# navi0105/LyricAlignment

Hardware: AMD Instinct MI355X
Metric: aligned audio-sec/sec (RTF^-1), Whisper-medium 30 s clips (higher is better)
Workload: dtype bf16; 1 GPU; whisper-medium encoder + BiGRU/FC head + CTC forced alignment, batch 32 x 30 s mel per GPU (BASELINE.json configs[1]); clips_per_gpu=32, frames=1500, vocab=21129, labels_per_clip=5..26 (one per sung note), pipeline=2 encoder stream(s) + 1 head stream, head over 4 batches

## Files before the change

### lyricalignment_amd/csrc/la_attention.hip

```cpp
#include <type_traits>

#include "la_common.h"

using la::bf16_t;

namespace {

typedef __attribute__((ext_vector_type(16))) float f32x16;
typedef __attribute__((ext_vector_type(8))) __bf16 bf16x8;
typedef __attribute__((ext_vector_type(8))) _Float16 f16x8;

template <typename T16> struct Half16;
template <> struct Half16<bf16_t> {
    typedef bf16x8 vec8;
    typedef __bf16 elem;
    static constexpr unsigned kOnes = 0x3F803F80u;
    static constexpr float kPLimit = 0x1p30f;
    __device__ static __forceinline__ f32x16 mfma32(vec8 a, vec8 b, f32x16 c) { return __builtin_amdgcn_mfma_f32_32x32x16_bf16(a, b, c, 0, 0, 0); }
};
template <> struct Half16<la::f16_t> {
    typedef f16x8 vec8;
    typedef _Float16 elem;
    static constexpr unsigned kOnes = 0x3C003C00u;
    static constexpr float kPLimit = 0x1p13f;
    __device__ static __forceinline__ f32x16 mfma32(vec8 a, vec8 b, f32x16 c) { return __builtin_amdgcn_mfma_f32_32x32x16_f16(a, b, c, 0, 0, 0); }
};
typedef __attribute__((ext_vector_type(4))) short s16x4;

constexpr int QT = 128;
constexpr int KT = 64;
constexpr float kLog2e = 1.4426950408889634f;

struct AttnParams {
    const void *q, *k, *v;
    int64_t ld_q, ld_kv;
    void *out;
    int64_t ld_out;
    int q_len, kv_len, n_head, causal;
    int64_t q_bs, kv_bs, out_bs;
    int batch;
    float defer_thr;
    float *lse = nullptr;
    float score_scale = 1.4426950408889634f;
};

struct BlockCoord { int qt, head, clip; };
__device__ __forceinline__ BlockCoord block_coord(int nq, int n_head, int batch) {
    const int L = blockIdx.x, pairs = n_head * batch;
    int pair, qt;
    if ((pairs & 7) == 0) {
        const int x = L & 7, idx = L >> 3;
        pair = x + 8 * (idx / nq);
        qt = idx % nq;
    } else {
        pair = L / nq;
        qt = L % nq;
    }
    return BlockCoord{qt, pair % n_head, pair / n_head};
}

__device__ __forceinline__ int acc_row(int reg, int h) { return (reg & 3) + 8 * (reg >> 2) + 4 * h; }

__device__ __forceinline__ void glds16(const void *g, void *l) {
    la::glds16(g, l);
}

__device__ __forceinline__ int kswz(int r) { return (r >> 1) & 7; }
__device__ __forceinline__ int vswz(int r) { return ((r >> 1) & 1) << 2; }

struct KvOff { unsigned k[2], v[2]; };
template <int PER>
__device__ __forceinline__ KvOff kv_offsets_bf16(int64_t ld, int key0, int T, int wave, int lane) {
    KvOff o;
    const int r8 = lane >> 3, ps = lane & 7;
#pragma unroll
    for (int i = 0; i < PER; ++i) {
        const int r = (wave * PER + i) * 8 + r8;
        int rr = key0 + r < T ? r : T - 1 - key0;
        o.k[i] = (unsigned)(rr * ld * 2) + ((ps ^ kswz(r)) << 4);
        o.v[i] = (unsigned)(rr * ld * 2) + ((ps ^ vswz(r)) << 4);
    }
    return o;
}
template <int PER>
__device__ __forceinline__ void stage_kv_bf16(const bf16_t *kbase, const bf16_t *vbase, int64_t ld, int key0, const KvOff &o,
                                              unsigned kl, unsigned vl, int wave) {
    const bf16_t *ks = kbase + (int64_t)key0 * ld, *vs = vbase + (int64_t)key0 * ld;
#pragma unroll
    for (int i = 0; i < PER; ++i) {
        la::glds16_so(o.k[i], ks, kl + (wave * PER + i) * 1024);
        la::glds16_so(o.v[i], vs, vl + (wave * PER + i) * 1024);
    }
}

template <typename T16, int NW = 4, bool MSUM = false, int KO = 0, bool OPT = false, int PRIO = 0, bool FOLD = false>
__global__ __launch_bounds__(64 * NW, FOLD ? 4 : 2) void attention_bf16_kernel(AttnParams p) {
    static_assert(!(OPT && MSUM), "the optimistic form tests the vector-pipe row sums");
    static_assert(!FOLD || OPT, "the log2-domain form is a variant of the optimistic one");
    constexpr int QT = 32 * NW, PER = 8 / NW;
    typedef Half16<T16> HT;
    typedef typename HT::vec8 vec8;
    __shared__ __attribute__((aligned(16))) unsigned char lds[2 * 2 * KT * 128];
    const int T = p.kv_len;
    const BlockCoord bc = block_coord((p.q_len + QT - 1) / QT, p.n_head, p.batch);
    const int qt = bc.qt, head = bc.head, clip = bc.clip;
    const int tid = threadIdx.x, lane = tid & 63;
    const int wave = __builtin_amdgcn_readfirstlane(tid >> 6);
    const int i32 = lane & 31, h = lane >> 5;
    const bf16_t *base = reinterpret_cast<const bf16_t *>(p.q) + (int64_t)clip * p.q_bs * p.ld_q + head * 64;
    const bf16_t *kbase = reinterpret_cast<const bf16_t *>(p.k) + (int64_t)clip * p.kv_bs * p.ld_kv + head * 64;
    const bf16_t *vbase = reinterpret_cast<const bf16_t *>(p.v) + (int64_t)clip * p.kv_bs * p.ld_kv + head * 64;

    int qrow = qt * QT + wave * 32 + i32;
    const bool q_valid = qrow < p.q_len;
    qrow = q_valid ? qrow : p.q_len - 1;
    uint4 qf[4];
#pragma unroll
    for (int c = 0; c < 4; ++c) qf[c] = *reinterpret_cast<const uint4 *>(base + (int64_t)qrow * p.ld_q + 16 * c + 8 * h);

    f32x16 o[2];
#pragma unroll
    for (int b = 0; b < 2; ++b)
#pragma unroll
        for (int r = 0; r < 16; ++r) o[b][r] = 0.f;
    float m_run = FOLD ? 0.f : -INFINITY, l_part = 0.f;
    int plain = FOLD ? 1 : 0;
    const float kScale = FOLD ? 1.0f : p.score_scale;
    f32x16 osum;
#pragma unroll
    for (int r = 0; r < 16; ++r) osum[r] = 0.f;
    const uint4 ones4 = uint4{HT::kOnes, HT::kOnes, HT::kOnes, HT::kOnes};

    int nkv = (T + KT - 1) / KT;
    const int nkv_all = nkv;
    if (p.causal) nkv = min(nkv, (min(p.q_len, (qt + 1) * QT) - 1) / KT + 1);
    const unsigned lds0 = __builtin_amdgcn_readfirstlane(la::lds_addr_u32(lds));
    const KvOff off_full = kv_offsets_bf16<PER>(p.ld_kv, 0, KT, wave, lane);
    const KvOff off_last = kv_offsets_bf16<PER>(p.ld_kv, (nkv_all - 1) * KT, T, wave, lane);
    stage_kv_bf16<PER>(kbase, vbase, p.ld_kv, 0, nkv_all == 1 ? off_last : off_full, lds0, lds0 + KT * 128, wave);
    asm volatile("s_waitcnt vmcnt(0)" ::: "memory");
#pragma unroll
    for (int c = 0; c < 4; ++c) {
        typedef unsigned u32x4 __attribute__((ext_vector_type(4)));
        u32x4 t = __builtin_bit_cast(u32x4, qf[c]);
        asm volatile("" : "+v"(t));
        qf[c] = __builtin_bit_cast(uint4, t);
    }
    __syncthreads();

    const int g = lane >> 4, q4 = (lane & 15) >> 2, pp = lane & 3;

    auto tile = [&](int t, auto curc) __attribute__((always_inline)) {
        constexpr int cur = decltype(curc)::value;
        const unsigned char *kl = lds + cur * (2 * KT * 128);
        const unsigned char *vl = kl + KT * 128;
        if (t + 1 < nkv && !(KO & 8)) {
            const unsigned nk = lds0 + (cur ^ 1) * (2 * KT * 128);
            stage_kv_bf16<PER>(kbase, vbase, p.ld_kv, (t + 1) * KT, t + 2 == nkv_all ? off_last : off_full, nk, nk + KT * 128, wave);
        }
        f32x16 s[2];
        typedef std::integral_constant<int, 0> Sub0;
        typedef std::integral_constant<int, 1> Sub1;
        typedef std::integral_constant<int, 2> SubBoth;
        auto scores = [&](auto serialc, auto whichc) {
            constexpr bool serial = decltype(serialc)::value;
            constexpr int lo = decltype(whichc)::value == 2 ? 0 : decltype(whichc)::value;
            constexpr int hi = decltype(whichc)::value == 2 ? 2 : lo + 1;
            uint4 kf[2][4];
#pragma unroll
            for (int sub = lo; sub < hi; ++sub)
#pragma unroll
                for (int r = 0; r < 16; ++r) s[sub][r] = 0.f;
            if constexpr (!serial) {
#pragma unroll
                for (int c = 0; c < 4; ++c)
#pragma unroll
                    for (int sub = lo; sub < hi; ++sub) {
                        const int row = sub * 32 + i32;
                        if constexpr (KO & 4) kf[sub][c] = qf[(c + sub) & 3];
                        else kf[sub][c] = *reinterpret_cast<const uint4 *>(kl + row * 128 + (((2 * c + h) ^ kswz(row)) << 4));
                    }
            }
#pragma unroll
            for (int c = 0; c < 4; ++c) {
                if constexpr (serial) {
#pragma unroll
                    for (int sub = lo; sub < hi; ++sub) {
                        const int row = sub * 32 + i32;
                        kf[sub][c] = *reinterpret_cast<const uint4 *>(kl + row * 128 + (((2 * c + h) ^ kswz(row)) << 4));
                    }
                }
// ... 65 lines not shown
#pragma unroll
                for (int j = 0; j < 8; ++j) pf[j] = (typename HT::elem)s[sub][8 * ks + j];
                if constexpr (MSUM) osum = HT::mfma32(__builtin_bit_cast(vec8, ones4), pf, osum);
#pragma unroll
                for (int b = 0; b < 2; ++b) {
                    const int key0 = sub * 32 + 16 * ks + 4 * (g >> 1);
                    const int slot = b * 4 + 2 * (g & 1) + (pp >> 1);
                    const int r0 = key0 + q4, r1 = key0 + 8 + q4;
                    typedef __attribute__((ext_vector_type(8))) short s16x8;
                    s16x8 vf;
                    if constexpr (KO & 2) vf = __builtin_bit_cast(s16x8, qf[(2 * sub + ks + b) & 3]);
                    else {
                        const s16x4 v0 = __builtin_amdgcn_ds_read_tr16_b64_v4i16(
                            (__attribute__((address_space(3))) s16x4 *)(vl + r0 * 128 + ((slot ^ vswz(r0)) << 4) + (pp & 1) * 8));
                        const s16x4 v1 = __builtin_amdgcn_ds_read_tr16_b64_v4i16(
                            (__attribute__((address_space(3))) s16x4 *)(vl + r1 * 128 + ((slot ^ vswz(r1)) << 4) + (pp & 1) * 8));
                        vf = __builtin_shufflevector(v0, v1, 0, 1, 2, 3, 4, 5, 6, 7);
                    }
                    if constexpr (KO & 16) o[b][2 * sub + ks] += (float)vf[0] + (float)vf[7] + (float)pf[0] + (float)pf[7];
                    else o[b] = HT::mfma32(__builtin_bit_cast(vec8, vf), pf, o[b]);
                }
            }
        };
        auto redo = [&](auto whichc) -> float {
            scores(std::true_type{}, whichc);
            const float m_new = fmaxf(m_run, tile_max(whichc));
            const float alpha = __builtin_amdgcn_exp2f(m_run - m_new);
            m_run = m_new;
            plain = 0;
            rescale(alpha);
            l_part *= alpha;
            return exponentials(m_new, whichc);
        };
        if constexpr (PRIO == 1 || PRIO == 2) __builtin_amdgcn_s_setprio(3);
        scores(std::false_type{}, SubBoth{});
        if constexpr (PRIO == 1 || PRIO == 2) __builtin_amdgcn_s_setprio(0);
        if constexpr (PRIO == 3) __builtin_amdgcn_s_setprio(3);
        if constexpr (OPT) {
            float ps0 = exponentials(m_run, Sub0{});
            if (__builtin_expect(__builtin_amdgcn_ballot_w64(!(ps0 <= HT::kPLimit)) != 0, 0)) ps0 = redo(Sub0{});
            l_part += ps0;
            float ps1 = exponentials(m_run, Sub1{});
            pv_sub(Sub0{});
            if (__builtin_expect(__builtin_amdgcn_ballot_w64(!(ps1 <= HT::kPLimit)) != 0, 0)) ps1 = redo(Sub1{});
            l_part += ps1;
            if constexpr (PRIO == 3) __builtin_amdgcn_s_setprio(0);
            if constexpr (PRIO == 2) __builtin_amdgcn_s_setprio(3);
            pv_sub(Sub1{});
            if constexpr (PRIO == 2) __builtin_amdgcn_s_setprio(0);
        } else {
            const float mx2 = tile_max(SubBoth{});
            float m_new = m_run, alpha = 1.0f;
            if (__builtin_amdgcn_ballot_w64(mx2 > m_run + p.defer_thr) != 0) {
                m_new = fmaxf(m_run, mx2);
                alpha = __builtin_amdgcn_exp2f(m_run - m_new);
            }
            m_run = m_new;
            const float ps = exponentials(m_new, SubBoth{});
            if constexpr (!MSUM) l_part = l_part * alpha + ps;
            if (__builtin_amdgcn_ballot_w64(alpha != 1.0f) != 0) rescale(alpha);
            pv_sub(Sub0{});
            pv_sub(Sub1{});
        }
        asm volatile("s_waitcnt vmcnt(0)" ::: "memory");
        if constexpr (!(KO & 32)) __syncthreads();
    };
    auto sweep = [&]() __attribute__((always_inline)) {
        for (int t = 0; t < nkv; t += 2) {
            tile(t, std::integral_constant<int, 0>{});
            if (t + 1 < nkv) tile(t + 1, std::integral_constant<int, 1>{});
        }
    };
    sweep();
    if constexpr (FOLD) {
        const float l0 = l_part + __shfl_xor(l_part, 32);
        if (__builtin_amdgcn_readfirstlane(__syncthreads_or(q_valid && !(l0 >= 0x1p-100f && l0 <= 0x1p100f)))) {
#pragma unroll
            for (int b = 0; b < 2; ++b)
#pragma unroll
                for (int r = 0; r < 16; ++r) o[b][r] = 0.f;
            m_run = -INFINITY; l_part = 0.f; plain = 0;
            stage_kv_bf16<PER>(kbase, vbase, p.ld_kv, 0, nkv_all == 1 ? off_last : off_full, lds0, lds0 + KT * 128, wave);
            asm volatile("s_waitcnt vmcnt(0)" ::: "memory");
            __syncthreads();
            sweep();
        }
    }

    const float l = MSUM ? osum[0] : l_part + __shfl_xor(l_part, 32);
    const float inv = 1.0f / l;
    if (q_valid) {
        bf16_t *orow = reinterpret_cast<bf16_t *>(p.out) + ((int64_t)clip * p.out_bs + qrow) * p.ld_out + head * 64;
#pragma unroll
        for (int b = 0; b < 2; ++b)
#pragma unroll
            for (int r4 = 0; r4 < 4; ++r4) {
                *reinterpret_cast<ushort4 *>(orow + 32 * b + 8 * r4 + 4 * h) =
                    la::Pack4<T16>::run(o[b][4 * r4 + 0] * inv, o[b][4 * r4 + 1] * inv, o[b][4 * r4 + 2] * inv, o[b][4 * r4 + 3] * inv);
            }
    }
}

__device__ __forceinline__ void stage_kv_f32(const float *kbase, const float *vbase, int64_t ld, int key0, int T,
                                             unsigned char *kl, unsigned char *vl, int wave, int lane) {
    const int r4 = lane >> 4, ps = lane & 15;
#pragma unroll
    for (int i = 0; i < 4; ++i) {
        const int piece = wave * 4 + i;
        const int r = piece * 4 + r4;
        int key = key0 + r;
        key = key < T ? key : T - 1;
        const int ls = ps ^ (r & 15);
        glds16(kbase + (int64_t)key * ld + (ls << 2), kl + piece * 1024);
        glds16(vbase + (int64_t)key * ld + (ls << 2), vl + piece * 1024);
    }
}
// ... 97 lines not shown
                }
            }
        asm volatile("s_waitcnt vmcnt(0)" ::: "memory");
        __syncthreads();
        cur ^= 1;
    }

    const float l = l_part + __shfl_xor(l_part, 32);
    const float inv = 1.0f / l;
    if (p.lse && q_valid && h == 0)
        p.lse[((int64_t)clip * p.n_head + head) * p.q_len + qrow] = fmaf(m_run, 0.6931471805599453f, __logf(l));
    if (q_valid) {
        float *orow = reinterpret_cast<float *>(p.out) + ((int64_t)clip * p.out_bs + qrow) * p.ld_out + head * 64;
#pragma unroll
        for (int b = 0; b < 2; ++b)
#pragma unroll
            for (int r4 = 0; r4 < 4; ++r4)
                *reinterpret_cast<float4 *>(orow + 32 * b + 8 * r4 + 4 * h) =
                    make_float4(o[b][4 * r4 + 0] * inv, o[b][4 * r4 + 1] * inv, o[b][4 * r4 + 2] * inv, o[b][4 * r4 + 3] * inv);
    }
}

}

static int attention_launch(int dtype_arg, AttnParams p, int batch, hipStream_t stream) {
    const int dtype = dtype_arg & 0xff;
    const bool qlog2 = dtype_arg & LA_Q_LOG2;
    if (qlog2 && dtype != LA_BF16 && dtype != LA_F16) {
        la::set_error("attention: LA_Q_LOG2 goes with the 16-bit kernels");
        return LA_EINVAL;
    }
    p.score_scale = qlog2 ? 1.0f : kLog2e;
    p.batch = batch;
    const char *thr_env = la::dev_env("LA_ATTN_THR");
    p.defer_thr = thr_env ? (float)atof(thr_env) : 8.0f;
    const dim3 grid(la::cdiv(p.q_len, QT) * p.n_head * batch), block(256);
    if (dtype == LA_BF16 || dtype == LA_F16) {
        la::TimerScope ts("attention_bf16", stream);
        const int nw_opt = la::opts().attn_nw;
        const int nw = nw_opt ? nw_opt : (p.q_len >= 1024 ? 8 : 4);
        const dim3 grid8(la::cdiv(p.q_len, 256) * p.n_head * batch), block8(512);
        const bool wide = nw == 8 && p.q_len >= 256;
#ifdef LA_EXPERIMENTS
        const char *opt_env = getenv("LA_ATTN_OPT"), *fold_env = getenv("LA_ATTN_FOLD");
        const bool no_opt = opt_env && atoi(opt_env) == 0, no_fold = fold_env && atoi(fold_env) == 0;
        if (wide && no_opt) {
            if (dtype == LA_F16) hipLaunchKernelGGL((attention_bf16_kernel<la::f16_t, 8>), grid8, block8, 0, stream, p);
            else hipLaunchKernelGGL((attention_bf16_kernel<bf16_t, 8>), grid8, block8, 0, stream, p);
        } else if (wide && dtype == LA_BF16 && qlog2 && no_fold) {
            hipLaunchKernelGGL((attention_bf16_kernel<bf16_t, 8, false, 0, true>), grid8, block8, 0, stream, p);
        } else if (!wide && getenv("LA_ATTN_MSUM")) {
            if (dtype == LA_F16) hipLaunchKernelGGL((attention_bf16_kernel<la::f16_t, 4, true>), grid, block, 0, stream, p);
            else hipLaunchKernelGGL((attention_bf16_kernel<bf16_t, 4, true>), grid, block, 0, stream, p);
        } else if (!wide && no_opt) {
            if (dtype == LA_F16) hipLaunchKernelGGL((attention_bf16_kernel<la::f16_t, 4>), grid, block, 0, stream, p);
            else hipLaunchKernelGGL((attention_bf16_kernel<bf16_t, 4>), grid, block, 0, stream, p);
        } else if (!wide && dtype == LA_BF16 && qlog2 && no_fold) {
            hipLaunchKernelGGL((attention_bf16_kernel<bf16_t, 4, false, 0, true>), grid, block, 0, stream, p);
        } else
#endif
#ifdef LA_ATTN_KNOCKOUT
        if (const char *ko = getenv("LA_ATTN_KO"); ko && !wide) {
            switch (atoi(ko)) {
#define LA_KO_CASE(n) case n: hipLaunchKernelGGL((attention_bf16_kernel<bf16_t, 4, false, n>), grid, block, 0, stream, p); break;
                LA_KO_CASE(1) LA_KO_CASE(2) LA_KO_CASE(4) LA_KO_CASE(6) LA_KO_CASE(8) LA_KO_CASE(14) LA_KO_CASE(16) LA_KO_CASE(17)
                LA_KO_CASE(7) LA_KO_CASE(15) LA_KO_CASE(30)
#undef LA_KO_CASE
#define LA_KO_OPT(n, ko) case n: { const char *pad = getenv("LA_ATTN_LDSPAD"); \
        hipLaunchKernelGGL((attention_bf16_kernel<bf16_t, 4, false, ko, true>), grid, block, pad ? atoi(pad) : 0, stream, p); } break;
                LA_KO_OPT(132, 32) LA_KO_OPT(140, 40) LA_KO_OPT(100, 0) LA_KO_OPT(101, 1) LA_KO_OPT(106, 6) LA_KO_OPT(108, 8) LA_KO_OPT(114, 14) LA_KO_OPT(116, 16) LA_KO_OPT(130, 30)
#undef LA_KO_OPT
#define LA_KO_PRIO(n, pr) case n: hipLaunchKernelGGL((attention_bf16_kernel<bf16_t, 4, false, 0, true, pr>), grid, block, 0, stream, p); break;
                LA_KO_PRIO(201, 1) LA_KO_PRIO(202, 2) LA_KO_PRIO(203, 3)
#undef LA_KO_PRIO
                default: hipLaunchKernelGGL((attention_bf16_kernel<bf16_t, 4>), grid, block, 0, stream, p);
            }
        } else
#endif
        if (wide) {
            if (dtype == LA_F16) hipLaunchKernelGGL((attention_bf16_kernel<la::f16_t, 8, false, 0, true>), grid8, block8, 0, stream, p);
            else if (qlog2) hipLaunchKernelGGL((attention_bf16_kernel<bf16_t, 8, false, 0, true, 0, true>), grid8, block8, 0, stream, p);
            else hipLaunchKernelGGL((attention_bf16_kernel<bf16_t, 8, false, 0, true>), grid8, block8, 0, stream, p);
        } else if (dtype == LA_F16) hipLaunchKernelGGL((attention_bf16_kernel<la::f16_t, 4, false, 0, true>), grid, block, 0, stream, p);
        else if (qlog2) hipLaunchKernelGGL((attention_bf16_kernel<bf16_t, 4, false, 0, true, 0, true>), grid, block, 0, stream, p);
        else hipLaunchKernelGGL((attention_bf16_kernel<bf16_t, 4, false, 0, true>), grid, block, 0, stream, p);
    } else {
        static la::DeviceOnce attr_once;
        if (attr_once.pending()) {
            LA_HIP(hipFuncSetAttribute(reinterpret_cast<const void *>(attention_f32_kernel),
                                       hipFuncAttributeMaxDynamicSharedMemorySize, 4 * KT * 256));
            attr_once.mark();
        }
        la::TimerScope ts("attention_f32", stream);
        hipLaunchKernelGGL(attention_f32_kernel, grid, block, 4 * KT * 256, stream, p);
    }
    LA_LAUNCH_CHECK();
    return LA_OK;
}

extern "C" int la_attention(int32_t dtype_arg, const void *qkv, int64_t ld_qkv, void *out, int64_t ld_out, int32_t batch,
                            int32_t frames, int32_t n_head, void *stream_) {
    hipStream_t stream = (hipStream_t)stream_;
    if (batch == 0 || frames == 0) return LA_OK;
    LA_CHECK_ARG(qkv && out && batch > 0 && frames > 0 && n_head > 0, "attention: bad arguments");
    const int dtype = dtype_arg & 0xff;
    LA_CHECK_ARG((dtype_arg & ~(0xff | LA_Q_LOG2)) == 0 && (dtype == LA_F32 || dtype == LA_BF16 || dtype == LA_F16), "attention: bad dtype");
    const int es = dtype == LA_F32 ? 4 : 2;
    LA_CHECK_ARG(ld_qkv >= 3 * n_head * 64 && ld_out >= n_head * 64, "attention: leading dimensions too small");
    LA_CHECK_ARG((ld_qkv * es) % 16 == 0 && (ld_out * es) % 16 == 0 && (uintptr_t)qkv % 16 == 0 && (uintptr_t)out % 16 == 0,
                 "attention: rows must be 16-byte aligned");
    const char *b = reinterpret_cast<const char *>(qkv);
    const int d = n_head * 64;
    AttnParams p{b, b + (int64_t)d * es, b + (int64_t)2 * d * es, ld_qkv, ld_qkv, out, ld_out, frames, frames, n_head, 0, frames, frames, frames, 0};
    return attention_launch(dtype_arg, p, batch, stream);
}

extern "C" int la_attention_ex(int32_t dtype_arg, const void *q, int64_t ld_q, const void *k, const void *v, int64_t ld_kv,
                               void *out, int64_t ld_out, int32_t batch, int32_t q_len, int32_t kv_len, int32_t n_head,
// ... 49 lines not shown
```

### lyricalignment_amd/csrc/la_common.h

```cpp
#pragma once
#include <hip/hip_runtime.h>
#include <stdint.h>
#include <stdio.h>
#include <stdlib.h>
#include <string.h>

#include "../../include/lyricalign.h"

namespace la {

char *err_buf();
void set_error(const char *fmt, ...);

enum { SCRATCH_SPLITK = 0, SCRATCH_COLSUM = 1, SCRATCH_X2 = 2 };
void *stream_scratch(hipStream_t stream, int purpose, size_t bytes);

#define LA_CHECK_ARG(cond, ...)                \
    do {                                       \
        if (!(cond)) {                         \
            la::set_error(__VA_ARGS__);        \
            return LA_EINVAL;                  \
        }                                      \
    } while (0)

#define LA_HIP(expr)                                                                     \
    do {                                                                                 \
        hipError_t _e = (expr);                                                          \
        if (_e != hipSuccess) {                                                          \
            la::set_error("%s:%d %s -> %s", __FILE__, __LINE__, #expr, hipGetErrorString(_e)); \
            return LA_EHIP;                                                              \
        }                                                                                \
    } while (0)

#define LA_LAUNCH_CHECK()                                                               \
    do {                                                                                \
        hipError_t _e = hipGetLastError();                                              \
        if (_e != hipSuccess) {                                                         \
            la::set_error("%s:%d launch -> %s", __FILE__, __LINE__, hipGetErrorString(_e)); \
            return LA_EHIP;                                                             \
        }                                                                               \
    } while (0)

struct Options {
    int gemm_tile = 0, gemm_loop = 0, gemm_splitk = 1, attn_nw = 0, gru_nw = 0, gru_fence = 0, gru_handoff = 0, gru_poll_delay = 0, viterbi_dpp = 1,
        head_clip_cap = 0, ln_fusion = 1, resid_split = 1, x2_inference = 1, gru_timeout_us = 0, gru_fault_step = 0, x2_small = 0;
};
Options &opts();
#ifdef LA_EXPERIMENTS
inline const char *dev_env(const char *name) { return getenv(name); }
#define LA_DEV_BIT(word, bits) ((word) & (bits))
#else
inline const char *dev_env(const char *) { return nullptr; }
#define LA_DEV_BIT(word, bits) false
#endif

struct DeviceOnce {
    unsigned long long done[4] = {0, 0, 0, 0};
    static int current() {
        int d = 0;
        if (hipGetDevice(&d) != hipSuccess) d = 0;
        return d & 255;
    }
    bool pending() const {
        const int d = current();
        return !((__atomic_load_n(&done[d >> 6], __ATOMIC_ACQUIRE) >> (d & 63)) & 1ull);
    }
    void mark() {
        const int d = current();
        __atomic_fetch_or(&done[d >> 6], 1ull << (d & 63), __ATOMIC_RELEASE);
    }
};

struct TimerScope {
    bool active;
    hipStream_t stream;
    TimerScope(const char *family, hipStream_t s, double work = 0.0);
    ~TimerScope();
};
// ... 178 lines not shown
```

### lyricalignment_amd/csrc/la_elementwise.hip

```cpp
#include "la_common.h"

using la::bf16_t;

namespace {

__device__ __forceinline__ float wave_max(float v) {
#pragma unroll
    for (int o = 32; o > 0; o >>= 1) v = fmaxf(v, __shfl_xor(v, o));
    return v;
}
__device__ __forceinline__ float wave_sum(float v) {
#pragma unroll
    for (int o = 32; o > 0; o >>= 1) v += __shfl_xor(v, o);
    return v;
}

__global__ __launch_bounds__(256) void emissions_from_logits_kernel(
    const float *logits, int64_t bs, int64_t rs, int frames, int vocab, int variant, const int32_t *labels,
    int labels_stride, const int32_t *n_labels, int max_labels, float *em, int64_t em_bs, int64_t em_rs) {
    __shared__ float red[8];
    const int row = blockIdx.x;
    const int b = row / frames, t = row % frames;
    const float *x = logits + (int64_t)b * bs + (int64_t)t * rs;
    const int c0 = variant == LA_VARIANT_CTC ? 1 : 0;
// ... 149 lines not shown
template <typename T16, int MAXV>
__global__ __launch_bounds__(256) void row_stats16_kernel(const T16 *x, int64_t ldx, int M, int d, float eps, float2 *stats) {
    const int row = blockIdx.x * 4 + (threadIdx.x >> 6);
    const int lane = threadIdx.x & 63;
    if (row >= M) return;
    const T16 *xr = x + (int64_t)row * ldx;
    float v[MAXV][8];
    float sum = 0.f;
#pragma unroll
    for (int i = 0; i < MAXV; ++i) {
        const int c = (lane + 64 * i) * 8;
        if (c < d) {
            const uint4 raw = *reinterpret_cast<const uint4 *>(xr + c);
            const T16 *e = reinterpret_cast<const T16 *>(&raw);
#pragma unroll
            for (int j = 0; j < 8; ++j) { v[i][j] = la::Elem<T16>::load(e + j); sum += v[i][j]; }
        } else {
#pragma unroll
            for (int j = 0; j < 8; ++j) v[i][j] = 0.f;
        }
    }
    const float mean = wave_sum(sum) / (float)d;
    float sq = 0.f;
#pragma unroll
    for (int i = 0; i < MAXV; ++i) {
        const int c = (lane + 64 * i) * 8;
        if (c < d) {
#pragma unroll
            for (int j = 0; j < 8; ++j) { const float a = v[i][j] - mean; sq = fmaf(a, a, sq); }
        }
    }
    const float var = wave_sum(sq) / (float)d;
    if (lane == 0) stats[row] = make_float2(mean, 1.0f / sqrtf(var + eps));
}

__global__ void cast_f32_bf16_kernel(const float *x, bf16_t *y, int64_t n) {
    int64_t i = ((int64_t)blockIdx.x * blockDim.x + threadIdx.x) * 4;
    const int64_t stride = (int64_t)gridDim.x * blockDim.x * 4;
    for (; i + 3 < n; i += stride) {
        const float4 v = *reinterpret_cast<const float4 *>(x + i);
        ushort4 pk;
        pk.x = la::f32_to_bf16(v.x); pk.y = la::f32_to_bf16(v.y);
        pk.z = la::f32_to_bf16(v.z); pk.w = la::f32_to_bf16(v.w);
        *reinterpret_cast<ushort4 *>(y + i) = pk;
    }
    if (blockIdx.x == 0 && threadIdx.x == 0)
        for (int64_t j = n & ~(int64_t)3; j < n; ++j) y[j] = la::f32_to_bf16(x[j]);
}

__global__ void cast_bf16_f32_kernel(const bf16_t *x, float *y, int64_t n) {
    int64_t i = (int64_t)blockIdx.x * blockDim.x + threadIdx.x;
    const int64_t stride = (int64_t)gridDim.x * blockDim.x;
    for (; i < n; i += stride) y[i] = la::bf16_to_f32(x[i]);
}

template <typename TOut>
__global__ __launch_bounds__(256) void mel_to_rows_kernel(const float *mel, int64_t mbs, int64_t mrs, int n_mels,
                                                          int frames, TOut *out, int c_pad) {
    __shared__ float tile[32][33];
    const int b = blockIdx.z;
    const int t0 = blockIdx.x * 32;
    const int c0 = blockIdx.y * 32;
    const int tx = threadIdx.x & 31, ty = threadIdx.x >> 5;
    for (int i = ty; i < 32; i += 8) {
        const int c = c0 + i, r = t0 + tx;
        const int t = r - 1;
// ... 84 lines not shown
    const unsigned char *l = reinterpret_cast<const unsigned char *>(lo);
    if (out_dtype == LA_F32)
        hipLaunchKernelGGL((layernorm_split_kernel<T16, float, 8>), grid, block, 0, stream, h, l, ldx, M, d, gamma, beta, (float *)y, ldy);
    else if (out_dtype == LA_F16)
        hipLaunchKernelGGL((layernorm_split_kernel<T16, la::f16_t, 8>), grid, block, 0, stream, h, l, ldx, M, d, gamma, beta, (la::f16_t *)y, ldy);
    else
        hipLaunchKernelGGL((layernorm_split_kernel<T16, bf16_t, 8>), grid, block, 0, stream, h, l, ldx, M, d, gamma, beta, (bf16_t *)y, ldy);
    LA_LAUNCH_CHECK();
    return LA_OK;
}

extern "C" int la_layernorm_split(int32_t dtype, const void *hi, const void *lo, int64_t ldx, int32_t M, int32_t d, const float *gamma,
                                  const float *beta, void *y, int64_t ldy, int32_t out_dtype, void *stream_) {
    hipStream_t stream = (hipStream_t)stream_;
    if (M == 0) return LA_OK;
    LA_CHECK_ARG(hi && lo && gamma && beta && y, "layernorm_split: null pointer");
    LA_CHECK_ARG(dtype == LA_BF16 || dtype == LA_F16, "layernorm_split: the stream's hi part is bf16 or f16");
    LA_CHECK_ARG(d > 0 && d % 4 == 0 && d <= 64 * 4 * 8 && ldx % 4 == 0 && ldy % 4 == 0 && (uintptr_t)hi % 8 == 0 && (uintptr_t)lo % 4 == 0,
                 "layernorm_split: d=%d unsupported or misaligned rows", d);
    LA_CHECK_ARG(out_dtype == LA_F32 || out_dtype == LA_BF16 || out_dtype == LA_F16, "layernorm_split: bad dtype");
    la::TimerScope ts("layernorm", stream);
    return dtype == LA_F16 ? layernorm_split_launch<la::f16_t>(hi, lo, ldx, M, d, gamma, beta, y, ldy, out_dtype, stream)
                           : layernorm_split_launch<bf16_t>(hi, lo, ldx, M, d, gamma, beta, y, ldy, out_dtype, stream);
}

extern "C" int la_row_stats16(int32_t dtype, const void *x, int64_t ldx, int32_t M, int32_t d, float eps, float *stats, void *stream_) {
    if (M == 0) return LA_OK;
    LA_CHECK_ARG(x && stats && M > 0 && d > 0, "row_stats16: bad arguments");
    LA_CHECK_ARG(dtype == LA_BF16 || dtype == LA_F16, "row_stats16: 16-bit rows only");
    LA_CHECK_ARG(d % 8 == 0 && d <= 64 * 8 * 4 && ldx % 8 == 0 && ((uintptr_t)x % 16 == 0) && ((uintptr_t)stats % 8 == 0),
                 "row_stats16: d must be a multiple of 8 and <= 2048, rows 16-byte aligned");
    hipStream_t stream = (hipStream_t)stream_;
    la::TimerScope ts("layernorm", stream);
    const dim3 grid(la::cdiv(M, 4)), block(256);
    if (dtype == LA_F16)
        hipLaunchKernelGGL((row_stats16_kernel<la::f16_t, 4>), grid, block, 0, stream, (const la::f16_t *)x, ldx, M, d, eps, (float2 *)stats);
    else
        hipLaunchKernelGGL((row_stats16_kernel<bf16_t, 4>), grid, block, 0, stream, (const bf16_t *)x, ldx, M, d, eps, (float2 *)stats);
    LA_LAUNCH_CHECK();
    return LA_OK;
}

extern "C" int la_cast_f32_to_bf16(const float *x, void *y, int64_t n, void *stream_) {
    if (n == 0) return LA_OK;
    LA_CHECK_ARG(x && y && n > 0, "cast: bad arguments");
    LA_CHECK_ARG(((uintptr_t)x % 16 == 0) && ((uintptr_t)y % 8 == 0), "cast: pointers must be 16/8-byte aligned");
    const int grid = (int)std::min<int64_t>(2048, la::cdiv(n, 1024));
    hipLaunchKernelGGL(cast_f32_bf16_kernel, dim3(grid), dim3(256), 0, (hipStream_t)stream_, x, (bf16_t *)y, n);
    LA_LAUNCH_CHECK();
    return LA_OK;
}

extern "C" int la_cast_bf16_to_f32(const void *x, float *y, int64_t n, void *stream_) {
    if (n == 0) return LA_OK;
    LA_CHECK_ARG(x && y && n > 0, "cast: bad arguments");
    const int grid = (int)std::min<int64_t>(2048, la::cdiv(n, 256));
    hipLaunchKernelGGL(cast_bf16_f32_kernel, dim3(grid), dim3(256), 0, (hipStream_t)stream_, (const bf16_t *)x, y, n);
    LA_LAUNCH_CHECK();
    return LA_OK;
}

extern "C" int la_mel_to_rows(const float *mel, int64_t mel_batch_stride, int64_t mel_row_stride, int32_t batch,
                              int32_t n_mels, int32_t frames, void *out, int32_t c_pad, int32_t dtype, void *stream_) {
    if (batch == 0) return LA_OK;
    LA_CHECK_ARG(mel && out && batch > 0 && n_mels > 0 && frames > 0 && c_pad >= n_mels, "mel_to_rows: bad arguments");
    LA_CHECK_ARG(dtype == LA_F32 || dtype == LA_BF16 || dtype == LA_F16, "mel_to_rows: bad dtype");
    const dim3 grid(la::cdiv(frames + 2, 32), la::cdiv(c_pad, 32), batch), block(256);
    hipStream_t stream = (hipStream_t)stream_;
    if (dtype == LA_F32)
        hipLaunchKernelGGL((mel_to_rows_kernel<float>), grid, block, 0, stream, mel, mel_batch_stride, mel_row_stride,
                           n_mels, frames, (float *)out, c_pad);
// ... 100 lines not shown
```

### lyricalignment_amd/csrc/la_runtime.cpp

```cpp
#include <stdarg.h>
#include <stdlib.h>

#include <mutex>
#include <string>
#include <vector>

#include "la_common.h"

namespace la {

char *err_buf() {
    static thread_local char buf[512] = {0};
    return buf;
}

void set_error(const char *fmt, ...) {
    va_list ap;
    va_start(ap, fmt);
    vsnprintf(err_buf(), 512, fmt, ap);
    va_end(ap);
}

void *stream_scratch(hipStream_t stream, int purpose, size_t bytes) {
    struct Slot { int dev; hipStream_t stream; int purpose; void *ptr; size_t bytes; };
    static std::mutex mu;
    static std::vector<Slot> slots;
    int dev = 0;
    if (hipGetDevice(&dev) != hipSuccess) return nullptr;
    std::lock_guard<std::mutex> lock(mu);
    for (Slot &sl : slots)
        if (sl.dev == dev && sl.stream == stream && sl.purpose == purpose) {
            if (sl.bytes >= bytes) return sl.ptr;
            if (hipStreamSynchronize(stream) != hipSuccess) return nullptr;
            (void)hipFree(sl.ptr);
            sl.ptr = nullptr; sl.bytes = 0;
            if (hipMalloc(&sl.ptr, bytes) != hipSuccess) return nullptr;
            sl.bytes = bytes;
            return sl.ptr;
        }
    Slot sl{dev, stream, purpose, nullptr, bytes < ((size_t)1 << 20) ? ((size_t)1 << 20) : bytes};
    if (hipMalloc(&sl.ptr, sl.bytes) != hipSuccess) return nullptr;
    slots.push_back(sl);
    return sl.ptr;
}

namespace {
struct OptionDesc { const char *name, *env; int Options::*field; bool env_inverts; };
const OptionDesc kOptions[] = {
    {"gemm_tile", "LA_GEMM_TILE", &Options::gemm_tile, false},       {"gemm_loop", "LA_PP_DBG", &Options::gemm_loop, false},
    {"gemm_splitk", "LA_GEMM_NO_SPLITK", &Options::gemm_splitk, true}, {"attn_nw", "LA_ATTN_NW", &Options::attn_nw, false},
    {"gru_nw", "LA_GRU_NW", &Options::gru_nw, false},                 {"gru_fence", "LA_GRU_FENCE", &Options::gru_fence, false},
    {"gru_handoff", "LA_GRU_HANDOFF", &Options::gru_handoff, false}, {"gru_poll_delay", "LA_GRU_POLL_DELAY", &Options::gru_poll_delay, false},
    {"viterbi_dpp", "LA_VITERBI_NO_DPP", &Options::viterbi_dpp, true}, {"head_clip_cap", "LA_HEAD_CLIP_CAP", &Options::head_clip_cap, false},
    {"ln_fusion", "LA_LN_FUSION", &Options::ln_fusion, false},       {"resid_split", "LA_RESID_SPLIT", &Options::resid_split, false},
    {"x2_inference", "LA_X2_INFERENCE", &Options::x2_inference, false}, {"x2_small", "LA_X2_SMALL", &Options::x2_small, false},
    {"gru_timeout_us", "LA_GRU_TIMEOUT_US", &Options::gru_timeout_us, false}, {"gru_fault_step", "LA_GRU_FAULT_STEP", &Options::gru_fault_step, false},
};
}

Options &opts() {
    static Options o = [] {
        Options v;
        for (const OptionDesc &d : kOptions) {
            const char *e = getenv(d.env);
            if (!e) continue;
            v.*(d.field) = d.env_inverts ? 0 : atoi(e);
        }
        return v;
    }();
    return o;
}

namespace {
struct TimerState {
    std::mutex mu;
    bool enabled = false;
    std::string family;
    std::vector<std::pair<hipEvent_t, hipEvent_t>> pairs;
    std::vector<std::pair<hipEvent_t, hipEvent_t>> pool;
    int period = 1;
    int64_t seen = 0;
    double work = 0.0;
};
TimerState &ts() {
    static TimerState s;
    return s;
}
}

// ... 135 lines not shown
```

Before: 23640 audio-sec/sec.

## Skip dead query waves and half-empty last KV tile in attention; add optional ring buffer

Attention waves whose query rows all lie past q_len now only take part in staging and barriers and skip score, softmax and PV work. When the final KV tile holds at most 32 valid keys, only its first 32-key half is computed. Both are on by default and aim to remove padded work at the sequence tails, which matters for the 1500-frame encoder. Two opt-in paths are added but stay off by default: a three-slot LDS ring for K/V prefetch with partial vmcnt waits, and a multi-row LayerNorm statistics kernel. The extra template modes increase code size and add branches.

```diff
diff --git a/lyricalignment_amd/csrc/la_attention.hip b/lyricalignment_amd/csrc/la_attention.hip
--- a/lyricalignment_amd/csrc/la_attention.hip
+++ b/lyricalignment_amd/csrc/la_attention.hip
@@ -42,6 +42,7 @@
     float defer_thr;
     float *lse = nullptr;
     float score_scale = 1.4426950408889634f;
+    int tails = 1;
 };
 
 struct BlockCoord { int qt, head, clip; };
@@ -93,14 +94,15 @@
     }
 }
 
-template <typename T16, int NW = 4, bool MSUM = false, int KO = 0, bool OPT = false, int PRIO = 0, bool FOLD = false>
+template <typename T16, int NW = 4, bool MSUM = false, int KO = 0, bool OPT = false, int PRIO = 0, bool FOLD = false, int RING = 2>
 __global__ __launch_bounds__(64 * NW, FOLD ? 4 : 2) void attention_bf16_kernel(AttnParams p) {
     static_assert(!(OPT && MSUM), "the optimistic form tests the vector-pipe row sums");
     static_assert(!FOLD || OPT, "the log2-domain form is a variant of the optimistic one");
+    static_assert(RING == 2 || RING == 3, "double buffer or ring of three");
     constexpr int QT = 32 * NW, PER = 8 / NW;
     typedef Half16<T16> HT;
     typedef typename HT::vec8 vec8;
-    __shared__ __attribute__((aligned(16))) unsigned char lds[2 * 2 * KT * 128];
+    __shared__ __attribute__((aligned(16))) unsigned char lds[RING * 2 * KT * 128];
     const int T = p.kv_len;
     const BlockCoord bc = block_coord((p.q_len + QT - 1) / QT, p.n_head, p.batch);
     const int qt = bc.qt, head = bc.head, clip = bc.clip;
@@ -114,6 +116,7 @@
     int qrow = qt * QT + wave * 32 + i32;
     const bool q_valid = qrow < p.q_len;
     qrow = q_valid ? qrow : p.q_len - 1;
+    const bool live = !p.tails || qt * QT + wave * 32 < p.q_len;
     uint4 qf[4];
 #pragma unroll
     for (int c = 0; c < 4; ++c) qf[c] = *reinterpret_cast<const uint4 *>(base + (int64_t)qrow * p.ld_q + 16 * c + 8 * h);
@@ -137,8 +140,13 @@
     const unsigned lds0 = __builtin_amdgcn_readfirstlane(la::lds_addr_u32(lds));
     const KvOff off_full = kv_offsets_bf16<PER>(p.ld_kv, 0, KT, wave, lane);
     const KvOff off_last = kv_offsets_bf16<PER>(p.ld_kv, (nkv_all - 1) * KT, T, wave, lane);
-    stage_kv_bf16<PER>(kbase, vbase, p.ld_kv, 0, nkv_all == 1 ? off_last : off_full, lds0, lds0 + KT * 128, wave);
-    asm volatile("s_waitcnt vmcnt(0)" ::: "memory");
+    auto prologue = [&]() __attribute__((always_inline)) {
+        stage_kv_bf16<PER>(kbase, vbase, p.ld_kv, 0, nkv_all == 1 ? off_last : off_full, lds0, lds0 + KT * 128, wave);
+        if (RING == 3 && nkv > 1)
+            stage_kv_bf16<PER>(kbase, vbase, p.ld_kv, KT, nkv_all == 2 ? off_last : off_full, lds0 + 2 * KT * 128, lds0 + 3 * KT * 128, wave);
+        asm volatile("s_waitcnt vmcnt(0)" ::: "memory");
+    };
+    prologue();
 #pragma unroll
     for (int c = 0; c < 4; ++c) {
         typedef unsigned u32x4 __attribute__((ext_vector_type(4)));
@@ -150,13 +158,20 @@
 
     const int g = lane >> 4, q4 = (lane & 15) >> 2, pp = lane & 3;
 
-    auto tile = [&](int t, auto curc) __attribute__((always_inline)) {
-        constexpr int cur = decltype(curc)::value;
+    typedef std::integral_constant<int, 0> kFull;
+    typedef std::integral_constant<int, 1> kHalf;
+    typedef std::integral_constant<int, 2> kDead;
+    auto tile = [&](int t, auto curc, auto modec) __attribute__((always_inline)) {
+        constexpr int mode = decltype(modec)::value;
+        const int cur = curc;
         const unsigned char *kl = lds + cur * (2 * KT * 128);
         const unsigned char *vl = kl + KT * 128;
-        if (t + 1 < nkv && !(KO & 8)) {
-            const unsigned nk = lds0 + (cur ^ 1) * (2 * KT * 128);
-            stage_kv_bf16<PER>(kbase, vbase, p.ld_kv, (t + 1) * KT, t + 2 == nkv_all ? off_last : off_full, nk, nk + KT * 128, wave);
+        constexpr int AHEAD = RING - 1;
+        const int nxt = (cur + AHEAD) % RING;
+        const bool staged = t + AHEAD < nkv && !(KO & 8);
+        if (staged) {
+            const unsigned nk = lds0 + nxt * (2 * KT * 128);
+            stage_kv_bf16<PER>(kbase, vbase, p.ld_kv, (t + AHEAD) * KT, t + AHEAD + 1 == nkv_all ? off_last : off_full, nk, nk + KT * 128, wave);
         }
         f32x16 s[2];
         typedef std::integral_constant<int, 0> Sub0;
@@ -288,44 +303,77 @@
             l_part *= alpha;
             return exponentials(m_new, whichc);
         };
-        if constexpr (PRIO == 1 || PRIO == 2) __builtin_amdgcn_s_setprio(3);
-        scores(std::false_type{}, SubBoth{});
-        if constexpr (PRIO == 1 || PRIO == 2) __builtin_amdgcn_s_setprio(0);
-        if constexpr (PRIO == 3) __builtin_amdgcn_s_setprio(3);
-        if constexpr (OPT) {
-            float ps0 = exponentials(m_run, Sub0{});
-            if (__builtin_expect(__builtin_amdgcn_ballot_w64(!(ps0 <= HT::kPLimit)) != 0, 0)) ps0 = redo(Sub0{});
-            l_part += ps0;
-            float ps1 = exponentials(m_run, Sub1{});
-            pv_sub(Sub0{});
-            if (__builtin_expect(__builtin_amdgcn_ballot_w64(!(ps1 <= HT::kPLimit)) != 0, 0)) ps1 = redo(Sub1{});
-            l_part += ps1;
-            if constexpr (PRIO == 3) __builtin_amdgcn_s_setprio(0);
-            if constexpr (PRIO == 2) __builtin_amdgcn_s_setprio(3);
-            pv_sub(Sub1{});
-            if constexpr (PRIO == 2) __builtin_amdgcn_s_setprio(0);
-        } else {
-            const float mx2 = tile_max(SubBoth{});
+        auto textbook = [&](auto whichc) {
+            const float mx2 = tile_max(whichc);
             float m_new = m_run, alpha = 1.0f;
             if (__builtin_amdgcn_ballot_w64(mx2 > m_run + p.defer_thr) != 0) {
                 m_new = fmaxf(m_run, mx2);
                 alpha = __builtin_amdgcn_exp2f(m_run - m_new);
             }
             m_run = m_new;
-            const float ps = exponentials(m_new, SubBoth{});
+            const float ps = exponentials(m_new, whichc);
             if constexpr (!MSUM) l_part = l_part * alpha + ps;
             if (__builtin_amdgcn_ballot_w64(alpha != 1.0f) != 0) rescale(alpha);
             pv_sub(Sub0{});
-            pv_sub(Sub1{});
-        }
-        asm volatile("s_waitcnt vmcnt(0)" ::: "memory");
+            if constexpr (decltype(whichc)::value == 2) pv_sub(Sub1{});
+        };
+        if constexpr (mode == kHalf::value) {
+                        scores(std::false_type{}, Sub0{});
+            if constexpr (OPT) {
+                float ps0 = exponentials(m_run, Sub0{});
+                if (__builtin_expect(__builtin_amdgcn_ballot_w64(!(ps0 <= HT::kPLimit)) != 0, 0)) ps0 = redo(Sub0{});
+                l_part += ps0;
+                pv_sub(Sub0{});
+            } else {
+                textbook(Sub0{});
+            }
+        } else if constexpr (mode == kFull::value) {
+            if constexpr (PRIO == 1 || PRIO == 2) __builtin_amdgcn_s_setprio(3);
+            scores(std::false_type{}, SubBoth{});
+            if constexpr (PRIO == 1 || PRIO == 2) __builtin_amdgcn_s_setprio(0);
+            if constexpr (PRIO == 3) __builtin_amdgcn_s_setprio(3);
+            if constexpr (OPT) {
+                float ps0 = exponentials(m_run, Sub0{});
+                if (__builtin_expect(__builtin_amdgcn_ballot_w64(!(ps0 <= HT::kPLimit)) != 0, 0)) ps0 = redo(Sub0{});
+                l_part += ps0;
+                float ps1 = exponentials(m_run, Sub1{});
+                pv_sub(Sub0{});
+                if (__builtin_expect(__builtin_amdgcn_ballot_w64(!(ps1 <= HT::kPLimit)) != 0, 0)) ps1 = redo(Sub1{});
+                l_part += ps1;
+                if constexpr (PRIO == 3) __builtin_amdgcn_s_setprio(0);
+                if constexpr (PRIO == 2) __builtin_amdgcn_s_setprio(3);
+                pv_sub(Sub1{});
+                if constexpr (PRIO == 2) __builtin_amdgcn_s_setprio(0);
+            } else {
+                textbook(SubBoth{});
+            }
+        }
+        if (RING == 3 && staged) {
+            if constexpr (PER == 1) asm volatile("s_waitcnt vmcnt(2)" ::: "memory");
+            else asm volatile("s_waitcnt vmcnt(4)" ::: "memory");
+            static_assert(PER == 1 || PER == 2, "vmcnt(2 * PER)");
+        } else {
+            asm volatile("s_waitcnt vmcnt(0)" ::: "memory");
+        }
         if constexpr (!(KO & 32)) __syncthreads();
     };
+    auto run = [&](int t0, int t1, auto modec) __attribute__((always_inline)) {
+        for (int t = t0; t < t1; t += RING) {
+            tile(t, std::integral_constant<int, 0>{}, modec);
+            if (t + 1 < t1) tile(t + 1, std::integral_constant<int, 1>{}, modec);
+            if constexpr (RING == 3) {
+                if (t + 2 < t1) tile(t + 2, std::integral_constant<int, 2>{}, modec);
+            }
+        }
+    };
+    const int nfull = p.tails && nkv == nkv_all && T - (nkv - 1) * KT <= 32 ? nkv - 1 : nkv;
     auto sweep = [&]() __attribute__((always_inline)) {
-        for (int t = 0; t < nkv; t += 2) {
-            tile(t, std::integral_constant<int, 0>{});
-            if (t + 1 < nkv) tile(t + 1, std::integral_constant<int, 1>{});
-        }
+        if (!live) {
+            run(0, nkv, kDead{});
+            return;
+        }
+        run(0, nfull, kFull{});
+        if (nfull < nkv) tile(nfull, nfull % RING, kHalf{});
     };
     sweep();
     if constexpr (FOLD) {
@@ -336,8 +384,7 @@
 #pragma unroll
                 for (int r = 0; r < 16; ++r) o[b][r] = 0.f;
             m_run = -INFINITY; l_part = 0.f; plain = 0;
-            stage_kv_bf16<PER>(kbase, vbase, p.ld_kv, 0, nkv_all == 1 ? off_last : off_full, lds0, lds0 + KT * 128, wave);
-            asm volatile("s_waitcnt vmcnt(0)" ::: "memory");
+            prologue();
             __syncthreads();
             sweep();
         }
@@ -501,6 +548,7 @@
     }
     p.score_scale = qlog2 ? 1.0f : kLog2e;
     p.batch = batch;
+    p.tails = la::opts().attn_tails != 0;
     const char *thr_env = la::dev_env("LA_ATTN_THR");
     p.defer_thr = thr_env ? (float)atof(thr_env) : 8.0f;
     const dim3 grid(la::cdiv(p.q_len, QT) * p.n_head * batch), block(256);
@@ -546,13 +594,22 @@
             }
         } else
 #endif
-        if (wide) {
-            if (dtype == LA_F16) hipLaunchKernelGGL((attention_bf16_kernel<la::f16_t, 8, false, 0, true>), grid8, block8, 0, stream, p);
-            else if (qlog2) hipLaunchKernelGGL((attention_bf16_kernel<bf16_t, 8, false, 0, true, 0, true>), grid8, block8, 0, stream, p);
-            else hipLaunchKernelGGL((attention_bf16_kernel<bf16_t, 8, false, 0, true>), grid8, block8, 0, stream, p);
-        } else if (dtype == LA_F16) hipLaunchKernelGGL((attention_bf16_kernel<la::f16_t, 4, false, 0, true>), grid, block, 0, stream, p);
-        else if (qlog2) hipLaunchKernelGGL((attention_bf16_kernel<bf16_t, 4, false, 0, true, 0, true>), grid, block, 0, stream, p);
-        else hipLaunchKernelGGL((attention_bf16_kernel<bf16_t, 4, false, 0, true>), grid, block, 0, stream, p);
+        {
+#define LA_ATTN_WIDE(T16, FOLD)                                                                                                   \
+    do {                                                                                                                          \
+        if (ring3) hipLaunchKernelGGL((attention_bf16_kernel<T16, 8, false, 0, true, 0, FOLD, 3>), grid8, block8, 0, stream, p);  \
+        else hipLaunchKernelGGL((attention_bf16_kernel<T16, 8, false, 0, true, 0, FOLD, 2>), grid8, block8, 0, stream, p);        \
+    } while (0)
+            const bool ring3 = la::opts().attn_ring == 3;
+            if (wide) {
+                if (dtype == LA_F16) LA_ATTN_WIDE(la::f16_t, false);
+                else if (qlog2) LA_ATTN_WIDE(bf16_t, true);
+                else LA_ATTN_WIDE(bf16_t, false);
+            } else if (dtype == LA_F16) hipLaunchKernelGGL((attention_bf16_kernel<la::f16_t, 4, false, 0, true>), grid, block, 0, stream, p);
+            else if (qlog2) hipLaunchKernelGGL((attention_bf16_kernel<bf16_t, 4, false, 0, true, 0, true>), grid, block, 0, stream, p);
+            else hipLaunchKernelGGL((attention_bf16_kernel<bf16_t, 4, false, 0, true>), grid, block, 0, stream, p);
+#undef LA_ATTN_WIDE
+        }
     } else {
         static la::DeviceOnce attr_once;
         if (attr_once.pending()) {
diff --git a/lyricalignment_amd/csrc/la_common.h b/lyricalignment_amd/csrc/la_common.h
--- a/lyricalignment_amd/csrc/la_common.h
+++ b/lyricalignment_amd/csrc/la_common.h
@@ -43,7 +43,8 @@
 
 struct Options {
     int gemm_tile = 0, gemm_loop = 0, gemm_splitk = 1, attn_nw = 0, gru_nw = 0, gru_fence = 0, gru_handoff = 0, gru_poll_delay = 0, viterbi_dpp = 1,
-        head_clip_cap = 0, ln_fusion = 1, resid_split = 1, x2_inference = 1, gru_timeout_us = 0, gru_fault_step = 0, x2_small = 0;
+        head_clip_cap = 0, ln_fusion = 1, resid_split = 1, x2_inference = 1, gru_timeout_us = 0, gru_fault_step = 0, x2_small = 0,
+        attn_tails = 1, attn_ring = 2, row_stats_form = 0;
 };
 Options &opts();
 #ifdef LA_EXPERIMENTS
diff --git a/lyricalignment_amd/csrc/la_elementwise.hip b/lyricalignment_amd/csrc/la_elementwise.hip
--- a/lyricalignment_amd/csrc/la_elementwise.hip
+++ b/lyricalignment_amd/csrc/la_elementwise.hip
@@ -205,6 +205,64 @@
     }
     const float var = wave_sum(sq) / (float)d;
     if (lane == 0) stats[row] = make_float2(mean, 1.0f / sqrtf(var + eps));
+}
+
+template <typename T16, int MAXV, int R>
+__global__ __launch_bounds__(256) void row_stats16_multi_kernel(const T16 *x, int64_t ldx, int M, int d, float eps, float2 *stats) {
+    const int lane = threadIdx.x & 63;
+    const int wave = __builtin_amdgcn_readfirstlane(blockIdx.x * 4 + (threadIdx.x >> 6)), nwave = gridDim.x * 4;
+    for (int row0 = wave * R; row0 < M; row0 += nwave * R) {
+        float v[R][MAXV][8];
+#pragma unroll
+        for (int r = 0; r < R; ++r) {
+            const T16 *xr = x + (int64_t)min(row0 + r, M - 1) * ldx;
+#pragma unroll
+            for (int i = 0; i < MAXV; ++i) {
+                const int c = (lane + 64 * i) * 8;
+                uint4 raw = make_uint4(0u, 0u, 0u, 0u);
+                if (c < d) raw = *reinterpret_cast<const uint4 *>(xr + c);
+                const T16 *e = reinterpret_cast<const T16 *>(&raw);
+#pragma unroll
+                for (int j = 0; j < 8; ++j) v[r][i][j] = la::Elem<T16>::load(e + j);
+            }
+        }
+        float sum[R], sq[R];
+#pragma unroll
+        for (int r = 0; r < R; ++r) {
+            sum[r] = 0.f;
+#pragma unroll
+            for (int i = 0; i < MAXV; ++i)
+                if ((lane + 64 * i) * 8 < d) {
+#pragma unroll
+                    for (int j = 0; j < 8; ++j) sum[r] += v[r][i][j];
+                }
+        }
+#pragma unroll
+        for (int o = 32; o > 0; o >>= 1)
+#pragma unroll
+            for (int r = 0; r < R; ++r) sum[r] += __shfl_xor(sum[r], o);
+#pragma unroll
+        for (int r = 0; r < R; ++r) {
+            const float mean = sum[r] / (float)d;
+            sum[r] = mean;
+            sq[r] = 0.f;
+#pragma unroll
+            for (int i = 0; i < MAXV; ++i)
+                if ((lane + 64 * i) * 8 < d) {
+#pragma unroll
+                    for (int j = 0; j < 8; ++j) { const float a = v[r][i][j] - mean; sq[r] = fmaf(a, a, sq[r]); }
+                }
+        }
+#pragma unroll
+        for (int o = 32; o > 0; o >>= 1)
+#pragma unroll
+            for (int r = 0; r < R; ++r) sq[r] += __shfl_xor(sq[r], o);
+#pragma unroll
+        for (int r = 0; r < R; ++r) {
+            const float var = sq[r] / (float)d;
+            if (lane == 0 && row0 + r < M) stats[row0 + r] = make_float2(sum[r], 1.0f / sqrtf(var + eps));
+        }
+    }
 }
 
 __global__ void cast_f32_bf16_kernel(const float *x, bf16_t *y, int64_t n) {
@@ -355,11 +413,20 @@
                  "row_stats16: d must be a multiple of 8 and <= 2048, rows 16-byte aligned");
     hipStream_t stream = (hipStream_t)stream_;
     la::TimerScope ts("layernorm", stream);
-    const dim3 grid(la::cdiv(M, 4)), block(256);
-    if (dtype == LA_F16)
-        hipLaunchKernelGGL((row_stats16_kernel<la::f16_t, 4>), grid, block, 0, stream, (const la::f16_t *)x, ldx, M, d, eps, (float2 *)stats);
-    else
-        hipLaunchKernelGGL((row_stats16_kernel<bf16_t, 4>), grid, block, 0, stream, (const bf16_t *)x, ldx, M, d, eps, (float2 *)stats);
+    const dim3 block(256);
+    if (la::opts().row_stats_form == 0) {
+        const dim3 grid(la::cdiv(M, 4));
+        if (dtype == LA_F16)
+            hipLaunchKernelGGL((row_stats16_kernel<la::f16_t, 4>), grid, block, 0, stream, (const la::f16_t *)x, ldx, M, d, eps, (float2 *)stats);
+        else
+            hipLaunchKernelGGL((row_stats16_kernel<bf16_t, 4>), grid, block, 0, stream, (const bf16_t *)x, ldx, M, d, eps, (float2 *)stats);
+    } else {
+        const dim3 grid(std::min(la::cdiv(M, 4 * 2), 256 * 8));
+#define LA_RS_MULTI(T16, MAXV) hipLaunchKernelGGL((row_stats16_multi_kernel<T16, MAXV, 2>), grid, block, 0, stream, (const T16 *)x, ldx, M, d, eps, (float2 *)stats)
+        if (dtype == LA_F16) { if (d > 1024) LA_RS_MULTI(la::f16_t, 4); else LA_RS_MULTI(la::f16_t, 2); }
+        else { if (d > 1024) LA_RS_MULTI(bf16_t, 4); else LA_RS_MULTI(bf16_t, 2); }
+#undef LA_RS_MULTI
+    }
     LA_LAUNCH_CHECK();
     return LA_OK;
 }
diff --git a/lyricalignment_amd/csrc/la_runtime.cpp b/lyricalignment_amd/csrc/la_runtime.cpp
--- a/lyricalignment_amd/csrc/la_runtime.cpp
+++ b/lyricalignment_amd/csrc/la_runtime.cpp
@@ -55,6 +55,8 @@
     {"ln_fusion", "LA_LN_FUSION", &Options::ln_fusion, false},       {"resid_split", "LA_RESID_SPLIT", &Options::resid_split, false},
     {"x2_inference", "LA_X2_INFERENCE", &Options::x2_inference, false}, {"x2_small", "LA_X2_SMALL", &Options::x2_small, false},
     {"gru_timeout_us", "LA_GRU_TIMEOUT_US", &Options::gru_timeout_us, false}, {"gru_fault_step", "LA_GRU_FAULT_STEP", &Options::gru_fault_step, false},
+    {"attn_tails", "LA_ATTN_TAILS", &Options::attn_tails, false},     {"attn_ring", "LA_ATTN_RING", &Options::attn_ring, false},
+    {"row_stats_form", "LA_ROW_STATS_FORM", &Options::row_stats_form, false},
 };
 }
 
```

Result: no change. 23770 audio-sec/sec, median of 6 (+0.5%).
